# NVlabs/nvbio

Hardware: NVIDIA H100
Metric: Mreads/s (150bp) seed+extend (higher is better)
Workload: dtype int32

## Files before the change

nvbio_b200/csrc/gotoh_kernels.cu:

```cuda
#include "gotoh_core.cuh"
#include <atomic>
#include "../../include/nvbio_b200_debug.h"
#include "gotoh_full_core.cuh"
#include "pipeline_core.cuh"

namespace nvb {

static int g_traceback_fast = 1;
static int g_pair_extra_smem = 0;
static int g_pair_rows2 = 1;
static bool g_pair_fmt_ok = true;

constexpr int PAIR_BLOCKDIM    = 128;
constexpr int GENERIC_BLOCKDIM = 128;

struct GotohBatch {
    StrSet   pat, txt;
    const uint8_t* quals;
    const uint32_t* d_n;
    uint32_t n_max;
    int32_t* score;
    uint2*   sink;
};

// ... 15 lines not shown
            b.txt.words, b.txt.bits, b.txt.big_endian, str_off(b.txt, a), str_len(b.txt, a));
        b.score[a] = r.score;
        b.sink[a]  = make_uint2(r.x, r.y);
    }
}

template <int B, int TYPE>
__global__ void __launch_bounds__(GENERIC_BLOCKDIM)
gotoh_best2_kernel(const GotohScheme S, const GotohBatch b, uint32_t distinct_dist, int32_t* __restrict__ out6)
{
    const uint32_t n = batch_count(b);
    const uint32_t a = blockIdx.x * GENERIC_BLOCKDIM + threadIdx.x;
    if (a >= n) return;
    Best2 b2; b2.init(distinct_dist);
    gotoh_generic_impl<B, TYPE, false>(S, b.pat.words, b.pat.bits, b.pat.big_endian, str_off(b.pat, a), str_len(b.pat, a), b.quals,
                                       b.txt.words, b.txt.bits, b.txt.big_endian, str_off(b.txt, a), str_len(b.txt, a), nullptr, &b2);
    int32_t* o = out6 + 6 * (size_t)a;
    o[0] = b2.s1; o[1] = (int32_t)b2.x1; o[2] = (int32_t)b2.y1; o[3] = b2.s2; o[4] = (int32_t)b2.x2; o[5] = (int32_t)b2.y2;
}
template <int B, int TYPE>
static int launch_best2(const GotohScheme& S, const GotohBatch& b, uint32_t distinct_dist, int32_t* out6, cudaStream_t s)
{
    gotoh_best2_kernel<B, TYPE><<<(b.n_max + GENERIC_BLOCKDIM - 1) / GENERIC_BLOCKDIM, GENERIC_BLOCKDIM, 0, s>>>(S, b, distinct_dist, out6);
    NVB_LAUNCH_CHECK();
    return NVB_OK;
}

__device__ __forceinline__ uint32_t swap_2bit_order(uint32_t x) {
    const uint32_t r = __brev(x);
    return ((r >> 1) & 0x55555555u) | ((r & 0x55555555u) << 1);
}

template <int B, int TYPE, int PFMT, bool ROWS2>
__global__ void __launch_bounds__(PAIR_BLOCKDIM, 4)
gotoh_pair_kernel(const GotohScheme S, const GotohBatch b, uint32_t sel_rows, uint32_t* __restrict__ todo, uint32_t* __restrict__ todo_count)
{
    extern __shared__ uint16_t sel_smem[];
    __shared__ uint32_t prof_tab[256];
    for (uint32_t q = threadIdx.x; q < 256u; q += PAIR_BLOCKDIM) prof_tab[q] = sub_profile(q, S.match - S.pgo, S.mismatch - S.pgo);
    __syncthreads();
    const uint32_t n = batch_count(b);
    const uint32_t n_pairs = (n + 1u) / 2u;
    uint16_t* my_sel = sel_smem + threadIdx.x;
    {
        const uint32_t pair = blockIdx.x * PAIR_BLOCKDIM + threadIdx.x;
        if (pair >= n_pairs) return;
        const uint32_t a0 = 2u * pair;
        const bool has1 = (a0 + 1u < n);
        const uint32_t a1 = has1 ? a0 + 1u : a0;

        const uint32_t M0 = str_len(b.pat, a0), M1 = str_len(b.pat, a1);
        const uint32_t N0 = str_len(b.txt, a0), N1 = str_len(b.txt, a1);
        const uint32_t Mmax = M0 > M1 ? M0 : M1;
        const uint32_t L = Mmax + (uint32_t)B - 1u;

        const bool ok = (M0 >= 1u) && (M1 >= 1u) && (N0 >= M0 + (uint32_t)B - 1u) && (N1 >= M1 + (uint32_t)B - 1u) &&
                        (L <= sel_rows) && (TYPE == NVB_LOCAL || M0 == M1);
        if (!ok) {
            const uint32_t cnt = has1 ? 2u : 1u;
            const uint32_t slot = atomicAdd(todo_count, cnt);
            todo[slot] = a0;
            if (has1) todo[slot + 1u] = a1;
            return;
        }

        {
            const uint32_t t0 = str_off(b.txt, a0), t1 = str_off(b.txt, a1);
            const uint32_t* __restrict__ w = b.txt.words;
            const bool be = b.txt.big_endian != 0;
            const uint32_t w0 = t0 >> 4, w1 = t1 >> 4;
            const uint32_t sh0 = 2u * (t0 & 15u), sh1 = 2u * (t1 & 15u);
            const uint32_t last0 = (t0 + N0 - 1u) >> 4, last1 = (t1 + N1 - 1u) >> 4;
            const uint32_t nw = (L + 15u) >> 4;
            for (uint32_t kb = 0; kb < nw; kb += 8u) {
                uint32_t a0[9], a1[9];
#pragma unroll
                for (uint32_t q = 0; q < 9u; ++q) {
                    a0[q] = (w0 + kb + q <= last0) ? w[w0 + kb + q] : 0u;
                    a1[q] = (w1 + kb + q <= last1) ? w[w1 + kb + q] : 0u;
                }
#pragma unroll
                for (uint32_t q = 0; q < 8u; ++q) {
                    const uint32_t k = kb + q;
                    if (k < nw) {
                        uint32_t c0, c1;
                        if (be) {
                            c0 = sh0 ? ((a0[q] << sh0) | (a0[q + 1] >> (32u - sh0))) : a0[q];
                            c1 = sh1 ? ((a1[q] << sh1) | (a1[q + 1] >> (32u - sh1))) : a1[q];
                        } else {
                            c0 = sh0 ? ((a0[q] >> sh0) | (a0[q + 1] << (32u - sh0))) : a0[q];
                            c1 = sh1 ? ((a1[q] >> sh1) | (a1[q + 1] << (32u - sh1))) : a1[q];
                        }
                        const uint32_t first = k << 4;
                        const uint32_t v0 = N0 > first ? (N0 - first < 16u ? N0 - first : 16u) : 0u;
                        const uint32_t v1 = N1 > first ? (N1 - first < 16u ? N1 - first : 16u) : 0u;
                        const uint32_t m0 = v0 >= 16u ? 0xFFFFFFFFu : (be ? ~(0xFFFFFFFFu >> (2u * v0)) : ((1u << (2u * v0)) - 1u));
                        const uint32_t m1 = v1 >= 16u ? 0xFFFFFFFFu : (be ? ~(0xFFFFFFFFu >> (2u * v1)) : ((1u << (2u * v1)) - 1u));
                        c0 &= m0; c1 &= m1;
                        if (!be) { c0 = swap_2bit_order(c0); c1 = swap_2bit_order(c1); }
#pragma unroll
                        for (uint32_t by = 0; by < 4u; ++by) {
                            const uint32_t W = prmt(c0, c1, (3u - by) | ((7u - by) << 4) | 0x3200u);
#pragma unroll
                            for (uint32_t m = 0; m < 4u; ++m) {
                                const uint32_t x = (W >> (6u - 2u * m)) & 0x0303u;
                                my_sel[(first + 4u * by + m) * PAIR_BLOCKDIM] = (uint16_t)(x * 0x11u + 0xC480u);
                            }
                        }
                    }
                }
            }
        }

        SinkResult r0, r1;
        gotoh_pair<B, TYPE, PFMT, ROWS2>(S, b.pat.words, b.pat.bits, b.pat.big_endian,
                            str_off(b.pat, a0), M0, str_off(b.pat, a1), M1, N0, N1,
                            my_sel, PAIR_BLOCKDIM, r0, r1, b.quals, prof_tab);
        b.score[a0] = r0.score; b.sink[a0] = make_uint2(r0.x, r0.y);
        if (has1) { b.score[a1] = r1.score; b.sink[a1] = make_uint2(r1.x, r1.y); }
    }
}

template <int TYPE>
__global__ void __launch_bounds__(GENERIC_BLOCKDIM)
gotoh_full_kernel(const GotohScheme S, const GotohBatch b, int2* __restrict__ col)
{
    const uint32_t n = batch_count(b);
    const uint32_t a = blockIdx.x * GENERIC_BLOCKDIM + threadIdx.x;
    if (a >= n) return;
    const SinkResult r = gotoh_full<TYPE>(S, b.pat.words, b.pat.bits, b.pat.big_endian, str_off(b.pat, a), str_len(b.pat, a),
                                          b.txt.words, b.txt.bits, b.txt.big_endian, str_off(b.txt, a), str_len(b.txt, a),
                                          col + a, (size_t)b.n_max, b.quals);
    b.score[a] = r.score;
    b.sink[a]  = make_uint2(r.x, r.y);
}

struct WindowArgs { uint32_t wb, we; const int32_t* min_score; short2* ckpt; uint8_t* alive; };

template <int B, int TYPE>
__global__ void __launch_bounds__(GENERIC_BLOCKDIM)
gotoh_window_kernel(const GotohScheme S, const GotohBatch b, const WindowArgs w)
{
    const uint32_t n = batch_count(b);
    const uint32_t a = blockIdx.x * GENERIC_BLOCKDIM + threadIdx.x;
    if (a >= n) return;
    SinkResult r;
    if (w.wb == 0) { r.score = NVB_SINK_MIN; r.x = r.y = 0xFFFFFFFFu; b.score[a] = r.score; b.sink[a] = make_uint2(r.x, r.y); w.alive[a] = 1; }
    else { if (!w.alive[a]) return; r.score = b.score[a]; const uint2 k = b.sink[a]; r.x = k.x; r.y = k.y; }
    const uint32_t M = str_len(b.pat, a);
    if (w.wb >= M) return;
    const bool ok = gotoh_window<B, TYPE>(S, b.pat.words, b.pat.bits, b.pat.big_endian, str_off(b.pat, a), M, b.quals,
                                          b.txt.words, b.txt.bits, b.txt.big_endian, str_off(b.txt, a), str_len(b.txt, a),
// ... 361 lines not shown
    }
    const uint32_t lane = threadIdx.x & 31u, a0 = a - lane;
    const uint32_t wrote = __ballot_sync(0xffffffffu, done);
    for (uint32_t w = wrote; w; w &= w - 1u) {
        const uint32_t src = __ffs(w) - 1u;
        uint32_t m = __shfl_sync(0xffffffffu, len, src);
        m = m < o.max_ops ? m : o.max_ops;
        uint8_t* ops = o.ops + (size_t)(a0 + src) * o.max_ops;
        for (uint32_t i = lane; i < m; i += 32u) ops[i] = (uint8_t)DIR_SUB;
    }
}

template <int B, int TYPE>
static int launch_traceback(const GotohScheme& S, const GotohBatch& b, const TracebackOut& o, const uint32_t* todo, const uint32_t* todo_count, cudaStream_t s)
{
    const uint32_t grid = (b.n_max + GENERIC_BLOCKDIM - 1) / GENERIC_BLOCKDIM;
    gotoh_traceback_kernel<B, TYPE><<<grid, GENERIC_BLOCKDIM, 0, s>>>(S, b, o, todo, todo_count);
    NVB_LAUNCH_CHECK();
    return NVB_OK;
}

template <int B, int TYPE>
static int launch_generic(const GotohScheme& S, const GotohBatch& b, const uint32_t* todo, const uint32_t* todo_count, uint32_t n_hint, cudaStream_t s)
{
    uint32_t grid = (n_hint + GENERIC_BLOCKDIM - 1) / GENERIC_BLOCKDIM;
    const uint32_t cap = sm_count() * 32u;
    if (todo) grid = grid < cap ? grid : cap;
    if (grid == 0) grid = 1;
    gotoh_generic_kernel<B, TYPE><<<grid, GENERIC_BLOCKDIM, 0, s>>>(S, b, todo, todo_count);
    NVB_LAUNCH_CHECK();
    return NVB_OK;
}

template <int B, int TYPE, int PFMT, bool ROWS2>
static int launch_pair_fmt(const GotohScheme& S, const GotohBatch& b, uint32_t sel_rows, uint32_t* todo, uint32_t* todo_count, cudaStream_t s)
{
    const size_t smem = (size_t)((sel_rows + 15u) & ~15u) * PAIR_BLOCKDIM * sizeof(uint16_t) + (size_t)g_pair_extra_smem;
    static std::atomic<bool> attr_done[NVB_MAX_DEVICES];
    int dev = 0;
    NVB_CUDA_TRY(cudaGetDevice(&dev));
    if (dev < 0 || dev >= NVB_MAX_DEVICES) return NVB_E_UNSUPPORTED;
    if (!attr_done[dev].load(std::memory_order_acquire)) {
        NVB_CUDA_TRY(cudaFuncSetAttribute(gotoh_pair_kernel<B, TYPE, PFMT, ROWS2>, cudaFuncAttributeMaxDynamicSharedMemorySize, 200 * 1024));
        attr_done[dev].store(true, std::memory_order_release);
    }
    const uint32_t pairs = (b.n_max + 1u) / 2u;
    const uint32_t grid = (pairs + PAIR_BLOCKDIM - 1) / PAIR_BLOCKDIM;
    gotoh_pair_kernel<B, TYPE, PFMT, ROWS2><<<grid, PAIR_BLOCKDIM, smem, s>>>(S, b, sel_rows, todo, todo_count);
    NVB_LAUNCH_CHECK();
    return NVB_OK;
}
template <int B, int TYPE, int PFMT>
static int launch_pair_rows(const GotohScheme& S, const GotohBatch& b, uint32_t sel_rows, uint32_t* todo, uint32_t* todo_count, cudaStream_t s)
{
    if (g_pair_rows2) return launch_pair_fmt<B, TYPE, PFMT, true>(S, b, sel_rows, todo, todo_count, s);
    return launch_pair_fmt<B, TYPE, PFMT, false>(S, b, sel_rows, todo, todo_count, s);
}
template <int B, int TYPE>
static int launch_pair(const GotohScheme& S, const GotohBatch& b, uint32_t sel_rows, uint32_t* todo, uint32_t* todo_count, cudaStream_t s)
{
    if (!S.qtab && b.pat.big_endian && b.pat.bits == 2u && g_pair_fmt_ok) return launch_pair_rows<B, TYPE, 2>(S, b, sel_rows, todo, todo_count, s);
    if (!S.qtab && b.pat.big_endian && b.pat.bits == 4u && g_pair_fmt_ok) return launch_pair_rows<B, TYPE, 4>(S, b, sel_rows, todo, todo_count, s);
    return launch_pair_rows<B, TYPE, 0>(S, b, sel_rows, todo, todo_count, s);
}

#define NVB_TYPE_SWITCH(BAND, FN, ...)                                            \
    switch (type) {                                                               \
    case NVB_GLOBAL:      return FN<BAND, NVB_GLOBAL>(__VA_ARGS__);               \
    case NVB_LOCAL:       return FN<BAND, NVB_LOCAL>(__VA_ARGS__);                \
    case NVB_SEMI_GLOBAL: return FN<BAND, NVB_SEMI_GLOBAL>(__VA_ARGS__);          \
    default:              return NVB_E_INVALID; }

static int dispatch_generic(int band, int type, const GotohScheme& S, const GotohBatch& b, const uint32_t* todo, const uint32_t* todo_count, uint32_t n_hint, cudaStream_t s)
{
    switch (band) {
    case 3:  NVB_TYPE_SWITCH(3,  launch_generic, S, b, todo, todo_count, n_hint, s)
    case 5:  NVB_TYPE_SWITCH(5,  launch_generic, S, b, todo, todo_count, n_hint, s)
    case 7:  NVB_TYPE_SWITCH(7,  launch_generic, S, b, todo, todo_count, n_hint, s)
    case 15: NVB_TYPE_SWITCH(15, launch_generic, S, b, todo, todo_count, n_hint, s)
    case 31: NVB_TYPE_SWITCH(31, launch_generic, S, b, todo, todo_count, n_hint, s)
    case 63: NVB_TYPE_SWITCH(63, launch_generic, S, b, todo, todo_count, n_hint, s)
    }
    return NVB_E_INVALID;
// ... 30 lines not shown
static void set_route(int packed, const uint32_t* todo_count) { g_route_packed = packed; g_route_todo_count = todo_count; }

static int banded_impl(int band, int type, const nvb_gotoh_scheme* scheme,
                       const nvb_string_set* patterns, const uint8_t* d_quals, const nvb_string_set* texts,
                       const uint32_t* d_n, uint32_t n_max, int32_t* d_score, nvb_uint2* d_sink,
                       void* d_temp, size_t* temp_bytes, void* stream)
{
    if (!scheme || !temp_bytes || !valid_strset(patterns) || !valid_strset(texts)) return NVB_E_INVALID;
    if (!(band == 3 || band == 5 || band == 7 || band == 15 || band == 31 || band == 63)) return NVB_E_INVALID;
    if (type < 0 || type > 2) return NVB_E_INVALID;

    TempCarver tc(d_temp);
    uint32_t* todo_count = tc.take<uint32_t>(4);
    uint32_t* todo       = tc.take<uint32_t>((size_t)n_max + 2);
    const size_t need = tc.total();
    if (!d_temp || *temp_bytes < need) { *temp_bytes = need; return NVB_E_TEMP_SIZE; }
    if (n_max == 0) return NVB_OK;
    if (!d_score || !d_sink) return NVB_E_INVALID;

    cudaStream_t s = as_stream(stream);
    GotohBatch b;
    b.pat = make_strset(patterns); b.txt = make_strset(texts); b.quals = d_quals;
    b.d_n = d_n; b.n_max = n_max; b.score = d_score; b.sink = (uint2*)d_sink;
    const GotohScheme S = make_scheme(scheme);

    const uint32_t max_m = patterns->length;
    const uint32_t sel_rows = max_m + (uint32_t)band - 1u;
    const size_t smem = (size_t)((sel_rows + 15u) & ~15u) * PAIR_BLOCKDIM * sizeof(uint16_t);
    const bool fast = (g_force_path != 1) && texts->bits == 2 && max_m >= 1 && smem <= 200u * 1024u &&
                      pair_path_ok(band, type, scheme, max_m);
    if (!fast) { set_route(0, nullptr); return dispatch_generic(band, type, S, b, nullptr, nullptr, n_max, s); }

    set_route(1, todo_count);
    NVB_CUDA_TRY(cudaMemsetAsync(todo_count, 0, sizeof(uint32_t), s));
    int r = dispatch_pair(band, type, S, b, sel_rows, todo, todo_count, s);
    if (r != NVB_OK) return r;
    return dispatch_generic(band, type, S, b, todo, todo_count, n_max, s);
}

template <int TYPE, int W>
static int full_tb_launch(const FullTbArgs* a, uint32_t max_n, size_t* pool_bytes, cudaStream_t s)
{
    int per_sm = 0;
    NVB_CUDA_TRY(cudaOccupancyMaxActiveBlocksPerMultiprocessor(&per_sm, gotoh_full_warp_traceback_kernel<TYPE, W>, WARP_BLOCKDIM, 0));
    const uint32_t grid = sm_count() * (uint32_t)(per_sm > 0 ? per_sm : 1);
    const uint32_t slot_words = (max_n + 31u) * 32u * (uint32_t)FullTbLane<W>::NW;
    *pool_bytes = (size_t)grid * (WARP_BLOCKDIM / 32) * slot_words * sizeof(uint32_t);
    if (!a) return NVB_OK;
    gotoh_full_warp_traceback_kernel<TYPE, W><<<grid, WARP_BLOCKDIM, 0, s>>>(a->S, a->pat, a->txt, a->quals, a->score, a->sink, a->items,
                                                                            a->n_items, a->o, (uint32_t*)a->pool, slot_words);
    NVB_LAUNCH_CHECK();
    return NVB_OK;
}

int full_warp_traceback(int type, uint32_t max_m, uint32_t max_n, const FullTbArgs* a, size_t* pool_bytes, cudaStream_t s)
{
    if (max_m < 1u || max_m > FULL_TB_MAX_M || max_n > 65535u) return NVB_E_UNSUPPORTED;
#define NVB_TB_W(T)                                                                                                                 \
    switch ((max_m + 31u) / 32u) {                                                                                                  \
    case 1:  return full_tb_launch<T, 1>(a, max_n, pool_bytes, s);  case 2:  return full_tb_launch<T, 2>(a, max_n, pool_bytes, s);   \
    case 3:  return full_tb_launch<T, 3>(a, max_n, pool_bytes, s);  case 4:  return full_tb_launch<T, 4>(a, max_n, pool_bytes, s);   \
    case 5:  return full_tb_launch<T, 5>(a, max_n, pool_bytes, s);  case 6:  return full_tb_launch<T, 6>(a, max_n, pool_bytes, s);   \
    case 7:  return full_tb_launch<T, 7>(a, max_n, pool_bytes, s);  case 8:  return full_tb_launch<T, 8>(a, max_n, pool_bytes, s);   \
    case 9:  return full_tb_launch<T, 9>(a, max_n, pool_bytes, s);  case 10: return full_tb_launch<T, 10>(a, max_n, pool_bytes, s);  \
    case 11: return full_tb_launch<T, 11>(a, max_n, pool_bytes, s); case 12: return full_tb_launch<T, 12>(a, max_n, pool_bytes, s);  \
    case 13: return full_tb_launch<T, 13>(a, max_n, pool_bytes, s); case 14: return full_tb_launch<T, 14>(a, max_n, pool_bytes, s);  \
    case 15: return full_tb_launch<T, 15>(a, max_n, pool_bytes, s); default: return full_tb_launch<T, 16>(a, max_n, pool_bytes, s); }
// ... 346 lines not shown
```

nvbio_b200/csrc/pipeline.cu:

```cuda
#include "fm_core.cuh"
#include "gotoh_core.cuh"
#include "pipeline_core.cuh"
#include "gotoh_full_core.cuh"
#include <cub/agent/single_pass_scan_operators.cuh>
#include <cub/block/block_scan.cuh>
#include <cub/device/device_scan.cuh>
#include <cub/device/device_segmented_sort.cuh>
#include <mutex>

namespace nvb {

struct PipeGeom {
    uint32_t n_reads;
    uint32_t n_strings;
    uint32_t strands;
    uint32_t stride;
    uint32_t bits;
    uint32_t seeds_per_string;
    uint32_t seed_len, seed_interval;
    uint32_t band;
    uint32_t max_seed_hits;
    uint32_t genome_len;
};

// ... 172 lines not shown
    }
}

__global__ void __launch_bounds__(256)
pipe_expand_hits_kernel(const FmIndex f, const PipeGeom g, const uint2* __restrict__ ranges, const uint32_t* __restrict__ sizes,
                        const uint32_t* __restrict__ excl, const uint32_t* __restrict__ slen, const uint32_t* __restrict__ counts,
                        uint32_t* __restrict__ hit_string, uint32_t* __restrict__ p_off, uint32_t* __restrict__ p_len,
                        uint32_t* __restrict__ t_off, uint32_t* __restrict__ t_len)
{
    const uint32_t q = blockIdx.x * 256 + threadIdx.x;
    if (q >= g.n_strings * g.seeds_per_string) return;
    const uint32_t sz = sizes[q];
    if (sz == 0) return;
    const uint32_t base = excl[q], kept = counts[0];
    const uint32_t x = ranges[q].x;
    const uint32_t s = q / g.seeds_per_string, k = q % g.seeds_per_string;
    const uint32_t seed_begin = k * g.seed_interval;
    const uint32_t len = slen[s];
    for (uint32_t j = 0; j < sz; ++j) {
        const uint32_t h = base + j;
        if (h >= kept) break;
        const uint2 w = hit_window(fm_locate_one(f, x + j), seed_begin, len, g);
        hit_string[h] = s;
        p_off[h] = s * g.stride; p_len[h] = len;
        t_off[h] = w.x;          t_len[h] = w.y - w.x;
    }
}

struct Jobs { uint32_t *p_off, *p_len, *t_off, *t_len; };

constexpr uint32_t RJ_BLOCK = 128;
constexpr uint32_t RJ_STAGE = 640;
constexpr int      RJ_LOCAL = 6;
constexpr uint32_t RJ_CLAIMED = 0xFFFFFFFFu, RJ_CLAIMED_EMPTY = 0xFFFFFFFEu;
using RjTileState = cub::ScanTileState<uint32_t>;
using RjPrefixOp  = cub::TilePrefixCallbackOp<uint32_t, ::cuda::std::plus<uint32_t>, RjTileState>;

__global__ void __launch_bounds__(256)
pipe_resolve_init_kernel(RjTileState tiles, const uint32_t n_tiles, uint32_t* __restrict__ counts, uint32_t* __restrict__ dp_count)
{
    tiles.InitializeStatus((int)n_tiles);
    if (blockIdx.x == 0 && threadIdx.x == 0) { counts[2] = 0u; counts[3] = 0u; *dp_count = 0u; }
}

__global__ void __launch_bounds__(RJ_BLOCK, 8)
pipe_resolve_reads_kernel(const FmIndex f, const PipeGeom g, const uint2* __restrict__ ranges, const uint32_t* __restrict__ slen,
                          const uint32_t hit_capacity, RjTileState tiles, const uint32_t n_tiles, uint32_t* __restrict__ counts,
                          const int shortcut, const int32_t match, const int32_t mismatch, const int32_t max_gap_open,
                          const uint32_t* __restrict__ str_words, const uint32_t* __restrict__ genome,
                          uint32_t* __restrict__ j_string, uint32_t* __restrict__ j_first, const Jobs jobs,
                          int32_t* __restrict__ job_score, uint2* __restrict__ job_sink,
                          const Jobs dp, uint32_t* __restrict__ dp_job, uint32_t* __restrict__ dp_count,
                          unsigned long long* __restrict__ best_key, int32_t* best_score, uint32_t* best_pos, uint8_t* __restrict__ best_strand)
{
    using BlockScan = cub::BlockScan<uint32_t, RJ_BLOCK>;
    __shared__ struct { typename RjPrefixOp::TempStorage prefix; typename BlockScan::TempStorage scan; } s_tmp;
    __shared__ uint32_t st_string[RJ_STAGE], st_first[RJ_STAGE], st_toff[RJ_STAGE], st_tlen[RJ_STAGE], st_slot[RJ_STAGE];
    __shared__ unsigned long long s_key[RJ_BLOCK];
    __shared__ int32_t s_score[RJ_BLOCK];
    __shared__ uint32_t s_pos[RJ_BLOCK];
    __shared__ uint8_t s_strand[RJ_BLOCK];
    __shared__ uint32_t s_tile, s_cnt, s_base, s_dp_cnt, s_dp_base;
    if (threadIdx.x == 0) { s_tile = atomicAdd(counts + 3, 1u); s_cnt = 0u; s_dp_cnt = 0u; }
    s_key[threadIdx.x] = 0ull;
    __syncthreads();
    const uint32_t tile = s_tile, r0 = tile * RJ_BLOCK, r = r0 + threadIdx.x;
    const uint32_t per_read = g.strands * g.seeds_per_string;
    const bool live = r < g.n_reads;
    const uint2* rr = ranges + (size_t)r * per_read;

    uint32_t hits = 0, run = 0;
    if (live)
        for (uint32_t q = 0; q < per_read; ++q) hits += seed_range_hits(rr[q], g.max_seed_hits);
    if (tile == 0) {
        uint32_t aggregate;
        BlockScan(s_tmp.scan).ExclusiveSum(hits, run, aggregate);
        if (threadIdx.x == 0) tiles.SetInclusive(0, aggregate);
    } else {
        RjPrefixOp prefix(tiles, s_tmp.prefix, ::cuda::std::plus<uint32_t>{}, (int)tile);
        BlockScan(s_tmp.scan).ExclusiveSum(hits, run, prefix);
    }
    if (tile == n_tiles - 1u && threadIdx.x == RJ_BLOCK - 1u) {
        const uint32_t total = run + hits;
        counts[1] = total;
        counts[0] = total < hit_capacity ? total : hit_capacity;
    }

    if (live) {
        uint32_t lk_s[RJ_LOCAL], lk_b[RJ_LOCAL], lk_e[RJ_LOCAL];
        int n_local = 0;
        for (uint32_t strand = 0; strand < g.strands; ++strand) {
            const uint32_t s = r * g.strands + strand;
            const uint32_t len = slen[s];
            for (uint32_t k = 0; k < g.seeds_per_string; ++k) {
                const uint2 rq = rr[strand * g.seeds_per_string + k];
                const bool located = rq.y == 0xFFFFFFFFu;
                const uint32_t sz = seed_range_hits(rq, g.max_seed_hits);
                if (sz == 0u) continue;
                const uint32_t base = run, x = rq.x, seed_begin = k * g.seed_interval;
                run += sz;
                for (uint32_t j = 0; j < sz; ++j) {
                    const uint32_t h = base + j;
                    if (h >= hit_capacity) break;
                    const uint2 w = hit_window(located ? x : fm_locate_one(f, x + j), seed_begin, len, g);
                    bool seen = false;
#pragma unroll
                    for (int e = 0; e < RJ_LOCAL; ++e) seen |= (e < n_local) && lk_s[e] == s && lk_b[e] == w.x && lk_e[e] == w.y;
                    if (seen) continue;
#pragma unroll
                    for (int e = 0; e < RJ_LOCAL; ++e) if (e == n_local) { lk_s[e] = s; lk_b[e] = w.x; lk_e[e] = w.y; }
                    if (n_local < RJ_LOCAL) ++n_local;
                    const uint32_t slot = atomicAdd(&s_cnt, 1u);
                    if (slot < RJ_STAGE) { st_string[slot] = s; st_first[slot] = h; st_toff[slot] = w.x; st_tlen[slot] = w.y - w.x; }
                    else {
                        const uint32_t o = atomicAdd(counts + 2, 1u), d = atomicAdd(dp_count, 1u);
                        j_string[o] = s; j_first[o] = h;
                        jobs.p_off[o] = s * g.stride; jobs.p_len[o] = len; jobs.t_off[o] = w.x; jobs.t_len[o] = w.y - w.x;
                        dp.p_off[d] = s * g.stride; dp.p_len[d] = len; dp.t_off[d] = w.x; dp.t_len[d] = w.y - w.x; dp_job[d] = o;
                    }
                }
            }
        }
    }
    __syncthreads();

    const uint32_t n = s_cnt < RJ_STAGE ? s_cnt : RJ_STAGE;
    if (threadIdx.x == 0) s_base = n ? atomicAdd(counts + 2, n) : 0u;
    __syncthreads();
    for (uint32_t i = threadIdx.x; i < n; i += RJ_BLOCK) {
        const uint32_t o = s_base + i, s = st_string[i], first = st_first[i], len = slen[s], to = st_toff[i], N = st_tlen[i];
        j_string[o] = s; j_first[o] = first; jobs.p_off[o] = s * g.stride; jobs.p_len[o] = len; jobs.t_off[o] = to; jobs.t_len[o] = N;
        int32_t score = 0; uint32_t sx = 0, sy = 0;
        if (shortcut && gapless_job_shortcut(str_words, genome, s * g.stride, len, to, N, g.band, match, mismatch, max_gap_open, score, sx, sy,
                                             shortcut != 2)) {
            const uint2 sk = make_uint2(sx, sy);
            job_score[o] = score; job_sink[o] = sk;
            if (job_aligned(sk)) {
                st_slot[i] = RJ_CLAIMED; st_toff[i] = to + sx; st_tlen[i] = (uint32_t)score;
                atomicMax(&s_key[s / g.strands - r0], make_best_key(score, first));
            } else st_slot[i] = RJ_CLAIMED_EMPTY;
        } else st_slot[i] = atomicAdd(&s_dp_cnt, 1u);
    }
    __syncthreads();
    if (threadIdx.x == 0) s_dp_base = s_dp_cnt ? atomicAdd(dp_count, s_dp_cnt) : 0u;
    __syncthreads();
    for (uint32_t i = threadIdx.x; i < n; i += RJ_BLOCK) {
        const uint32_t slot = st_slot[i], s = st_string[i];
        if (slot == RJ_CLAIMED) {
            const uint32_t rl = s / g.strands - r0;
            const int32_t score = (int32_t)st_tlen[i];
            if (s_key[rl] == make_best_key(score, st_first[i])) { s_score[rl] = score; s_pos[rl] = st_toff[i]; s_strand[rl] = (uint8_t)(s % g.strands); }
// ... 1203 lines not shown
```

nvbio_b200/csrc/pipeline_core.cuh:

```cuda
#pragma once
#include "fm_core.cuh"

namespace nvb {

__host__ __device__ __forceinline__ uint32_t nvb_clz(uint32_t x) {
#ifdef __CUDA_ARCH__
    return (uint32_t)__clz((int)x);
#else
    return (uint32_t)__builtin_clz(x);
#endif
}

__host__ __device__ __forceinline__ uint32_t job_diff_bits(const uint32_t* __restrict__ str_words, const uint32_t* __restrict__ genome,
                                                           const uint32_t po, const uint32_t t, const uint32_t i, const uint32_t cnt)
{
    const uint32_t x = (be2_window(str_words, po + i, cnt) ^ be2_window(genome, t + i, cnt)) >> (32u - 2u * cnt);
    return (x | (x >> 1)) & 0x55555555u;
}
__host__ __device__ __forceinline__ uint32_t job_differences(const uint32_t* __restrict__ str_words, const uint32_t* __restrict__ genome,
                                                             const uint32_t po, const uint32_t M, const uint32_t t, const uint32_t limit)
{
    uint32_t mm = 0;
    for (uint32_t i = 0; i < M && mm <= limit; i += 16u) mm += nvb_popc(job_diff_bits(str_words, genome, po, t, i, M - i < 16u ? M - i : 16u));
    return mm;
}

__host__ __device__ __forceinline__ uint32_t diff_row_mask(const uint32_t w0, const uint32_t cnt, const uint32_t lo, const uint32_t hi)
{
    const uint32_t a = lo > w0 ? lo : w0, b = hi < w0 + cnt - 1u ? hi : w0 + cnt - 1u;
    if (a > b) return 0u;
    return ((2u << (2u * (w0 + cnt - 1u - a))) - 1u) & ~((1u << (2u * (w0 + cnt - 1u - b))) - 1u);
}
__host__ __device__ inline void job_diff_span(const uint32_t* __restrict__ str_words, const uint32_t* __restrict__ genome, const uint32_t po,
                                              const uint32_t t, const uint32_t lo, const uint32_t hi, int32_t& first, int32_t& last)
{
    first = (int32_t)hi + 1; last = (int32_t)lo - 1;
    for (uint32_t i = lo; i <= hi; i += 16u) {
        const uint32_t cnt = hi + 1u - i < 16u ? hi + 1u - i : 16u;
        const uint32_t d = job_diff_bits(str_words, genome, po, t, i, cnt);
        if (!d) continue;
        if (first > (int32_t)hi) first = (int32_t)(i + cnt - 1u - ((31u - nvb_clz(d)) >> 1));
        last = (int32_t)(i + cnt - 1u - ((31u - nvb_clz(d & (0u - d))) >> 1));
    }
}
__host__ __device__ __forceinline__ uint32_t text_window16(const uint32_t g0, const uint32_t g1, const uint32_t g2, const uint32_t g3, const uint32_t off)
{
    const uint32_t idx = off >> 4, sh = 2u * (off & 15u);
    const uint32_t hi = idx == 0u ? g0 : (idx == 1u ? g1 : g2), lo = idx == 0u ? g1 : (idx == 1u ? g2 : g3);
    return sh ? ((hi << sh) | (lo >> (32u - sh))) : hi;
}

__host__ __device__ inline bool gapless_job_shortcut(const uint32_t* __restrict__ str_words, const uint32_t* __restrict__ genome,
                                                     const uint32_t po, const uint32_t M, const uint32_t to, const uint32_t N, const uint32_t band,
                                                     const int32_t match, const int32_t mismatch, const int32_t max_gap_open,
                                                     int32_t& score, uint32_t& sink_x, uint32_t& sink_y, const bool one_gap = true)
{
    if (M < 1u || to == 0u || N < M + band - 1u) return false;
    const uint32_t j0 = band / 2u;
    const int32_t o = -max_gap_open, lim = !one_gap ? o : (o + match - mismatch < 2 * o ? o + match - mismatch : 2 * o);
    const uint32_t mm_max = (uint32_t)((lim - 1) / match);
    int32_t h = 0, best = 0, f1 = (int32_t)M, f2 = (int32_t)M, l1 = -1, l2 = -1; uint32_t end = 0, prev = 0, mm0 = 0;
    for (uint32_t i = 0; i < M && mm0 <= mm_max; i += 16u) {
        const uint32_t cnt = M - i < 16u ? M - i : 16u;
        uint32_t d = job_diff_bits(str_words, genome, po, to + j0, i, cnt);
        while (d && mm0 <= mm_max) {
            const uint32_t bit = 31u - nvb_clz(d);
            const uint32_t p = i + (cnt - 1u - (bit >> 1));
            d &= ~(1u << bit);
            h += match * (int32_t)(p - prev);
            if (h >= best) { best = h; end = p; }
            h += mismatch; h = h > 0 ? h : 0;
            if (mm0 == 0u) f1 = (int32_t)p; else if (mm0 == 1u) f2 = (int32_t)p;
            l2 = l1; l1 = (int32_t)p;
            prev = p + 1u; ++mm0;
        }
    }
    if (mm0 > mm_max) return false;
    h += match * (int32_t)(M - prev);
    if (h >= best) { best = h; end = M; }
    const int32_t delta = match * (int32_t)M - best;
    if (delta >= lim) return false;
    const bool gap1 = delta >= o;
    const uint32_t U = gap1 ? (uint32_t)((delta - o) / match) : 0u;
    if (gap1 && 2u * U + 1u > M) return false;
    const uint32_t hi = M - 1u - U;
    int32_t fa = f1 >= (int32_t)U ? f1 : (f2 >= (int32_t)U ? f2 : (int32_t)(M - U)), ba = l1 <= (int32_t)hi ? l1 : (l2 <= (int32_t)hi ? l2 : (int32_t)U - 1);
    fa = fa > (int32_t)hi ? (int32_t)(M - U) : fa; ba = ba < (int32_t)U ? (int32_t)U - 1 : ba;
    int32_t fb = INT_MIN, bb = INT_MAX; uint32_t fd = j0, bd = j0;
    const bool perfect = (mm0 == 0u);
    const uint32_t t = (uint32_t)(delta / match);
    const uint32_t c16 = M < 16u ? M : 16u;
    const uint32_t r0 = be2_window(str_words, po, c16) >> (32u - 2u * c16);
    const uint32_t wi = to >> 4, r = to & 15u, wl = (to + N - 1u) >> 4;
    const uint32_t g0 = genome[wi], g1 = (wi + 1u <= wl) ? genome[wi + 1u] : 0u;
    const uint32_t g2 = (wi + 2u <= wl) ? genome[wi + 2u] : 0u, g3 = (wi + 3u <= wl) ? genome[wi + 3u] : 0u;
    uint32_t rE = 0, e0 = 0, e1 = 0, e2 = 0, e3 = 0, mF = 0, mB = 0;
    const uint32_t te = to + M - c16, we = te >> 4;
    if (gap1) {
        rE = be2_window(str_words, po + M - c16, c16) >> (32u - 2u * c16);
        e0 = genome[we]; e1 = (we + 1u <= wl) ? genome[we + 1u] : 0u; e2 = (we + 2u <= wl) ? genome[we + 2u] : 0u; e3 = (we + 3u <= wl) ? genome[we + 3u] : 0u;
        mF = diff_row_mask(0u, c16, U, hi); mB = diff_row_mask(M - c16, c16, U, hi);
    }
    uint32_t jtop = j0;
    for (uint32_t jj = 0; jj < band; ++jj) {
        if (jj == j0) continue;
        const uint32_t x = (text_window16(g0, g1, g2, g3, r + jj) >> (32u - 2u * c16)) ^ r0, dx = (x | (x >> 1)) & 0x55555555u;
        if (gap1) {
// ... 176 lines not shown
```

Before: 400.2.

## Add persistent ticket scheduling to pair kernel, batch seed range loads, prefetch shortcut words

The pair Gotoh kernel gains a persistent-grid mode, used when the batch count lives on the device: warps claim 32 pairs at a time from an atomic ticket counter and the grid is capped at resident occupancy. The resolve-jobs kernel now loads seed ranges in vectorized batches and walks only non-empty ranges via bitmasks. The gapless shortcut prefetches read and genome words into registers and computes diffs inline instead of calling a per-16-base helper. Together these aim to cut wasted blocks, scalar loads and latency, at the cost of more register pressure and a second counter word that must be zeroed.

```diff
diff --git a/nvbio_b200/csrc/gotoh_kernels.cu b/nvbio_b200/csrc/gotoh_kernels.cu
--- a/nvbio_b200/csrc/gotoh_kernels.cu
+++ b/nvbio_b200/csrc/gotoh_kernels.cu
@@ -71,6 +71,86 @@
 }
 
 template <int B, int TYPE, int PFMT, bool ROWS2>
+__device__ __forceinline__ void gotoh_pair_job(const GotohScheme& S, const GotohBatch& b, const uint32_t sel_rows, uint32_t* __restrict__ todo,
+                                               uint32_t* __restrict__ todo_count, const uint32_t pair, const uint32_t n, uint16_t* my_sel,
+                                               const uint32_t* prof_tab)
+{
+    const uint32_t a0 = 2u * pair;
+    const bool has1 = (a0 + 1u < n);
+    const uint32_t a1 = has1 ? a0 + 1u : a0;
+
+    const uint32_t M0 = str_len(b.pat, a0), M1 = str_len(b.pat, a1);
+    const uint32_t N0 = str_len(b.txt, a0), N1 = str_len(b.txt, a1);
+    const uint32_t Mmax = M0 > M1 ? M0 : M1;
+    const uint32_t L = Mmax + (uint32_t)B - 1u;
+
+    const bool ok = (M0 >= 1u) && (M1 >= 1u) && (N0 >= M0 + (uint32_t)B - 1u) && (N1 >= M1 + (uint32_t)B - 1u) &&
+                    (L <= sel_rows) && (TYPE == NVB_LOCAL || M0 == M1);
+    if (!ok) {
+        const uint32_t cnt = has1 ? 2u : 1u;
+        const uint32_t slot = atomicAdd(todo_count, cnt);
+        todo[slot] = a0;
+        if (has1) todo[slot + 1u] = a1;
+        return;
+    }
+
+    {
+        const uint32_t t0 = str_off(b.txt, a0), t1 = str_off(b.txt, a1);
+        const uint32_t* __restrict__ w = b.txt.words;
+        const bool be = b.txt.big_endian != 0;
+        const uint32_t w0 = t0 >> 4, w1 = t1 >> 4;
+        const uint32_t sh0 = 2u * (t0 & 15u), sh1 = 2u * (t1 & 15u);
+        const uint32_t last0 = (t0 + N0 - 1u) >> 4, last1 = (t1 + N1 - 1u) >> 4;
+        const uint32_t nw = (L + 15u) >> 4;
+        for (uint32_t kb = 0; kb < nw; kb += 8u) {
+            uint32_t a0[9], a1[9];
+#pragma unroll
+            for (uint32_t q = 0; q < 9u; ++q) {
+                a0[q] = (w0 + kb + q <= last0) ? w[w0 + kb + q] : 0u;
+                a1[q] = (w1 + kb + q <= last1) ? w[w1 + kb + q] : 0u;
+            }
+#pragma unroll
+            for (uint32_t q = 0; q < 8u; ++q) {
+                const uint32_t k = kb + q;
+                if (k < nw) {
+                    uint32_t c0, c1;
+                    if (be) {
+                        c0 = sh0 ? ((a0[q] << sh0) | (a0[q + 1] >> (32u - sh0))) : a0[q];
+                        c1 = sh1 ? ((a1[q] << sh1) | (a1[q + 1] >> (32u - sh1))) : a1[q];
+                    } else {
+                        c0 = sh0 ? ((a0[q] >> sh0) | (a0[q + 1] << (32u - sh0))) : a0[q];
+                        c1 = sh1 ? ((a1[q] >> sh1) | (a1[q + 1] << (32u - sh1))) : a1[q];
+                    }
+                    const uint32_t first = k << 4;
+                    const uint32_t v0 = N0 > first ? (N0 - first < 16u ? N0 - first : 16u) : 0u;
+                    const uint32_t v1 = N1 > first ? (N1 - first < 16u ? N1 - first : 16u) : 0u;
+                    const uint32_t m0 = v0 >= 16u ? 0xFFFFFFFFu : (be ? ~(0xFFFFFFFFu >> (2u * v0)) : ((1u << (2u * v0)) - 1u));
+                    const uint32_t m1 = v1 >= 16u ? 0xFFFFFFFFu : (be ? ~(0xFFFFFFFFu >> (2u * v1)) : ((1u << (2u * v1)) - 1u));
+                    c0 &= m0; c1 &= m1;
+                    if (!be) { c0 = swap_2bit_order(c0); c1 = swap_2bit_order(c1); }
+#pragma unroll
+                    for (uint32_t by = 0; by < 4u; ++by) {
+                        const uint32_t W = prmt(c0, c1, (3u - by) | ((7u - by) << 4) | 0x3200u);
+#pragma unroll
+                        for (uint32_t m = 0; m < 4u; ++m) {
+                            const uint32_t x = (W >> (6u - 2u * m)) & 0x0303u;
+                            my_sel[(first + 4u * by + m) * PAIR_BLOCKDIM] = (uint16_t)(x * 0x11u + 0xC480u);
+                        }
+                    }
+                }
+            }
+        }
+    }
+
+    SinkResult r0, r1;
+    gotoh_pair<B, TYPE, PFMT, ROWS2>(S, b.pat.words, b.pat.bits, b.pat.big_endian,
+                        str_off(b.pat, a0), M0, str_off(b.pat, a1), M1, N0, N1,
+                        my_sel, PAIR_BLOCKDIM, r0, r1, b.quals, prof_tab);
+    b.score[a0] = r0.score; b.sink[a0] = make_uint2(r0.x, r0.y);
+    if (has1) { b.score[a1] = r1.score; b.sink[a1] = make_uint2(r1.x, r1.y); }
+}
+
+template <int B, int TYPE, int PFMT, bool ROWS2, bool TICKET>
 __global__ void __launch_bounds__(PAIR_BLOCKDIM, 4)
 gotoh_pair_kernel(const GotohScheme S, const GotohBatch b, uint32_t sel_rows, uint32_t* __restrict__ todo, uint32_t* __restrict__ todo_count)
 {
@@ -81,82 +161,19 @@
     const uint32_t n = batch_count(b);
     const uint32_t n_pairs = (n + 1u) / 2u;
     uint16_t* my_sel = sel_smem + threadIdx.x;
-    {
+    if (!TICKET) {
         const uint32_t pair = blockIdx.x * PAIR_BLOCKDIM + threadIdx.x;
         if (pair >= n_pairs) return;
-        const uint32_t a0 = 2u * pair;
-        const bool has1 = (a0 + 1u < n);
-        const uint32_t a1 = has1 ? a0 + 1u : a0;
-
-        const uint32_t M0 = str_len(b.pat, a0), M1 = str_len(b.pat, a1);
-        const uint32_t N0 = str_len(b.txt, a0), N1 = str_len(b.txt, a1);
-        const uint32_t Mmax = M0 > M1 ? M0 : M1;
-        const uint32_t L = Mmax + (uint32_t)B - 1u;
-
-        const bool ok = (M0 >= 1u) && (M1 >= 1u) && (N0 >= M0 + (uint32_t)B - 1u) && (N1 >= M1 + (uint32_t)B - 1u) &&
-                        (L <= sel_rows) && (TYPE == NVB_LOCAL || M0 == M1);
-        if (!ok) {
-            const uint32_t cnt = has1 ? 2u : 1u;
-            const uint32_t slot = atomicAdd(todo_count, cnt);
-            todo[slot] = a0;
-            if (has1) todo[slot + 1u] = a1;
-            return;
-        }
-
-        {
-            const uint32_t t0 = str_off(b.txt, a0), t1 = str_off(b.txt, a1);
-            const uint32_t* __restrict__ w = b.txt.words;
-            const bool be = b.txt.big_endian != 0;
-            const uint32_t w0 = t0 >> 4, w1 = t1 >> 4;
-            const uint32_t sh0 = 2u * (t0 & 15u), sh1 = 2u * (t1 & 15u);
-            const uint32_t last0 = (t0 + N0 - 1u) >> 4, last1 = (t1 + N1 - 1u) >> 4;
-            const uint32_t nw = (L + 15u) >> 4;
-            for (uint32_t kb = 0; kb < nw; kb += 8u) {
-                uint32_t a0[9], a1[9];
-#pragma unroll
-                for (uint32_t q = 0; q < 9u; ++q) {
-                    a0[q] = (w0 + kb + q <= last0) ? w[w0 + kb + q] : 0u;
-                    a1[q] = (w1 + kb + q <= last1) ? w[w1 + kb + q] : 0u;
-                }
-#pragma unroll
-                for (uint32_t q = 0; q < 8u; ++q) {
-                    const uint32_t k = kb + q;
-                    if (k < nw) {
-                        uint32_t c0, c1;
-                        if (be) {
-                            c0 = sh0 ? ((a0[q] << sh0) | (a0[q + 1] >> (32u - sh0))) : a0[q];
-                            c1 = sh1 ? ((a1[q] << sh1) | (a1[q + 1] >> (32u - sh1))) : a1[q];
-                        } else {
-                            c0 = sh0 ? ((a0[q] >> sh0) | (a0[q + 1] << (32u - sh0))) : a0[q];
-                            c1 = sh1 ? ((a1[q] >> sh1) | (a1[q + 1] << (32u - sh1))) : a1[q];
-                        }
-                        const uint32_t first = k << 4;
-                        const uint32_t v0 = N0 > first ? (N0 - first < 16u ? N0 - first : 16u) : 0u;
-                        const uint32_t v1 = N1 > first ? (N1 - first < 16u ? N1 - first : 16u) : 0u;
-                        const uint32_t m0 = v0 >= 16u ? 0xFFFFFFFFu : (be ? ~(0xFFFFFFFFu >> (2u * v0)) : ((1u << (2u * v0)) - 1u));
-                        const uint32_t m1 = v1 >= 16u ? 0xFFFFFFFFu : (be ? ~(0xFFFFFFFFu >> (2u * v1)) : ((1u << (2u * v1)) - 1u));
-                        c0 &= m0; c1 &= m1;
-                        if (!be) { c0 = swap_2bit_order(c0); c1 = swap_2bit_order(c1); }
-#pragma unroll
-                        for (uint32_t by = 0; by < 4u; ++by) {
-                            const uint32_t W = prmt(c0, c1, (3u - by) | ((7u - by) << 4) | 0x3200u);
-#pragma unroll
-                            for (uint32_t m = 0; m < 4u; ++m) {
-                                const uint32_t x = (W >> (6u - 2u * m)) & 0x0303u;
-                                my_sel[(first + 4u * by + m) * PAIR_BLOCKDIM] = (uint16_t)(x * 0x11u + 0xC480u);
-                            }
-                        }
-                    }
-                }
-            }
-        }
-
-        SinkResult r0, r1;
-        gotoh_pair<B, TYPE, PFMT, ROWS2>(S, b.pat.words, b.pat.bits, b.pat.big_endian,
-                            str_off(b.pat, a0), M0, str_off(b.pat, a1), M1, N0, N1,
-                            my_sel, PAIR_BLOCKDIM, r0, r1, b.quals, prof_tab);
-        b.score[a0] = r0.score; b.sink[a0] = make_uint2(r0.x, r0.y);
-        if (has1) { b.score[a1] = r1.score; b.sink[a1] = make_uint2(r1.x, r1.y); }
+        gotoh_pair_job<B, TYPE, PFMT, ROWS2>(S, b, sel_rows, todo, todo_count, pair, n, my_sel, prof_tab);
+    } else {
+        const uint32_t lane = threadIdx.x & 31u;
+        for (;;) {
+            uint32_t first = 0;
+            if (lane == 0u) first = atomicAdd(todo_count + 1, 32u);
+            first = __shfl_sync(0xFFFFFFFFu, first, 0);
+            if (first >= n_pairs) return;
+            if (first + lane < n_pairs) gotoh_pair_job<B, TYPE, PFMT, ROWS2>(S, b, sel_rows, todo, todo_count, first + lane, n, my_sel, prof_tab);
+        }
     }
 }
 
@@ -584,8 +601,8 @@
     return NVB_OK;
 }
 
-template <int B, int TYPE, int PFMT, bool ROWS2>
-static int launch_pair_fmt(const GotohScheme& S, const GotohBatch& b, uint32_t sel_rows, uint32_t* todo, uint32_t* todo_count, cudaStream_t s)
+template <int B, int TYPE, int PFMT, bool ROWS2, bool TICKET>
+static int launch_pair_grid(const GotohScheme& S, const GotohBatch& b, uint32_t sel_rows, uint32_t* todo, uint32_t* todo_count, cudaStream_t s)
 {
     const size_t smem = (size_t)((sel_rows + 15u) & ~15u) * PAIR_BLOCKDIM * sizeof(uint16_t) + (size_t)g_pair_extra_smem;
     static std::atomic<bool> attr_done[NVB_MAX_DEVICES];
@@ -593,14 +610,26 @@
     NVB_CUDA_TRY(cudaGetDevice(&dev));
     if (dev < 0 || dev >= NVB_MAX_DEVICES) return NVB_E_UNSUPPORTED;
     if (!attr_done[dev].load(std::memory_order_acquire)) {
-        NVB_CUDA_TRY(cudaFuncSetAttribute(gotoh_pair_kernel<B, TYPE, PFMT, ROWS2>, cudaFuncAttributeMaxDynamicSharedMemorySize, 200 * 1024));
+        NVB_CUDA_TRY(cudaFuncSetAttribute(gotoh_pair_kernel<B, TYPE, PFMT, ROWS2, TICKET>, cudaFuncAttributeMaxDynamicSharedMemorySize, 200 * 1024));
         attr_done[dev].store(true, std::memory_order_release);
     }
     const uint32_t pairs = (b.n_max + 1u) / 2u;
-    const uint32_t grid = (pairs + PAIR_BLOCKDIM - 1) / PAIR_BLOCKDIM;
-    gotoh_pair_kernel<B, TYPE, PFMT, ROWS2><<<grid, PAIR_BLOCKDIM, smem, s>>>(S, b, sel_rows, todo, todo_count);
+    uint32_t grid = (pairs + PAIR_BLOCKDIM - 1) / PAIR_BLOCKDIM;
+    if (TICKET) {
+        int per_sm = 0;
+        NVB_CUDA_TRY(cudaOccupancyMaxActiveBlocksPerMultiprocessor(&per_sm, gotoh_pair_kernel<B, TYPE, PFMT, ROWS2, TICKET>, PAIR_BLOCKDIM, smem));
+        const uint32_t resident = sm_count() * (uint32_t)(per_sm > 0 ? per_sm : 1);
+        grid = grid < resident ? grid : resident;
+    }
+    gotoh_pair_kernel<B, TYPE, PFMT, ROWS2, TICKET><<<grid, PAIR_BLOCKDIM, smem, s>>>(S, b, sel_rows, todo, todo_count);
     NVB_LAUNCH_CHECK();
     return NVB_OK;
+}
+template <int B, int TYPE, int PFMT, bool ROWS2>
+static int launch_pair_fmt(const GotohScheme& S, const GotohBatch& b, uint32_t sel_rows, uint32_t* todo, uint32_t* todo_count, cudaStream_t s)
+{
+    if (b.d_n) return launch_pair_grid<B, TYPE, PFMT, ROWS2, true>(S, b, sel_rows, todo, todo_count, s);
+    return launch_pair_grid<B, TYPE, PFMT, ROWS2, false>(S, b, sel_rows, todo, todo_count, s);
 }
 template <int B, int TYPE, int PFMT>
 static int launch_pair_rows(const GotohScheme& S, const GotohBatch& b, uint32_t sel_rows, uint32_t* todo, uint32_t* todo_count, cudaStream_t s)
@@ -697,7 +726,7 @@
     if (!fast) { set_route(0, nullptr); return dispatch_generic(band, type, S, b, nullptr, nullptr, n_max, s); }
 
     set_route(1, todo_count);
-    NVB_CUDA_TRY(cudaMemsetAsync(todo_count, 0, sizeof(uint32_t), s));
+    NVB_CUDA_TRY(cudaMemsetAsync(todo_count, 0, 2 * sizeof(uint32_t), s));
     int r = dispatch_pair(band, type, S, b, sel_rows, todo, todo_count, s);
     if (r != NVB_OK) return r;
     return dispatch_generic(band, type, S, b, todo, todo_count, n_max, s);
diff --git a/nvbio_b200/csrc/pipeline.cu b/nvbio_b200/csrc/pipeline.cu
--- a/nvbio_b200/csrc/pipeline.cu
+++ b/nvbio_b200/csrc/pipeline.cu
@@ -228,9 +228,35 @@
 constexpr uint32_t RJ_BLOCK = 128;
 constexpr uint32_t RJ_STAGE = 640;
 constexpr int      RJ_LOCAL = 6;
+constexpr uint32_t RJ_BATCH = 4;
 constexpr uint32_t RJ_CLAIMED = 0xFFFFFFFFu, RJ_CLAIMED_EMPTY = 0xFFFFFFFEu;
 using RjTileState = cub::ScanTileState<uint32_t>;
 using RjPrefixOp  = cub::TilePrefixCallbackOp<uint32_t, ::cuda::std::plus<uint32_t>, RjTileState>;
+
+template <uint32_t RB>
+__device__ __forceinline__ uint32_t range_batch(const uint2* __restrict__ rr, const uint32_t q0, const uint32_t n, const bool vec,
+                                                const uint32_t max_seed_hits, uint32_t& hits)
+{
+    uint2 v[RB];
+    if (vec) {
+#pragma unroll
+        for (uint32_t j = 0; j < RB; j += 2u) {
+            const uint4 w = q0 + j < n ? *reinterpret_cast<const uint4*>(rr + q0 + j) : make_uint4(1u, 0u, 1u, 0u);
+            v[j] = make_uint2(w.x, w.y); v[j + 1] = make_uint2(w.z, w.w);
+        }
+    } else {
+#pragma unroll
+        for (uint32_t j = 0; j < RB; ++j) v[j] = q0 + j < n ? rr[q0 + j] : make_uint2(1u, 0u);
+    }
+    uint32_t m = 0;
+#pragma unroll
+    for (uint32_t j = 0; j < RB; ++j) {
+        const uint32_t sz = seed_range_hits(v[j], max_seed_hits);
+        hits += sz;
+        m |= (sz != 0u ? 1u : 0u) << j;
+    }
+    return m;
+}
 
 __global__ void __launch_bounds__(256)
 pipe_resolve_init_kernel(RjTileState tiles, const uint32_t n_tiles, uint32_t* __restrict__ counts, uint32_t* __restrict__ dp_count)
@@ -265,9 +291,13 @@
     const bool live = r < g.n_reads;
     const uint2* rr = ranges + (size_t)r * per_read;
 
-    uint32_t hits = 0, run = 0;
+    const bool vec = ((per_read | (uint32_t)((size_t)ranges >> 3)) & 1u) == 0u;
+    uint32_t hits = 0, run = 0, nonempty = 0;
     if (live)
-        for (uint32_t q = 0; q < per_read; ++q) hits += seed_range_hits(rr[q], g.max_seed_hits);
+        for (uint32_t q0 = 0; q0 < per_read; q0 += 16u) {
+            const uint32_t m = range_batch<16>(rr, q0, per_read, vec, g.max_seed_hits, hits);
+            if (q0 < 32u) nonempty |= m << q0;
+        }
     if (tile == 0) {
         uint32_t aggregate;
         BlockScan(s_tmp.scan).ExclusiveSum(hits, run, aggregate);
@@ -285,34 +315,48 @@
     if (live) {
         uint32_t lk_s[RJ_LOCAL], lk_b[RJ_LOCAL], lk_e[RJ_LOCAL];
         int n_local = 0;
-        for (uint32_t strand = 0; strand < g.strands; ++strand) {
-            const uint32_t s = r * g.strands + strand;
-            const uint32_t len = slen[s];
-            for (uint32_t k = 0; k < g.seeds_per_string; ++k) {
-                const uint2 rq = rr[strand * g.seeds_per_string + k];
-                const bool located = rq.y == 0xFFFFFFFFu;
-                const uint32_t sz = seed_range_hits(rq, g.max_seed_hits);
-                if (sz == 0u) continue;
-                const uint32_t base = run, x = rq.x, seed_begin = k * g.seed_interval;
-                run += sz;
-                for (uint32_t j = 0; j < sz; ++j) {
-                    const uint32_t h = base + j;
-                    if (h >= hit_capacity) break;
-                    const uint2 w = hit_window(located ? x : fm_locate_one(f, x + j), seed_begin, len, g);
-                    bool seen = false;
+        const uint32_t len0 = slen[r * g.strands], len1 = g.strands > 1u ? slen[r * g.strands + 1u] : 0u;
+        for (uint32_t q0 = 0; q0 < per_read; q0 += 32u) {
+            uint32_t m = q0 ? 0u : nonempty, unused = 0;
+            if (q0)
+                for (uint32_t b = 0; b < 32u; b += 8u) m |= range_batch<8>(rr, q0 + b, per_read, vec, g.max_seed_hits, unused) << b;
+            while (m) {
+                uint32_t bq[RJ_BATCH], nb = 0;
+                uint2 brq[RJ_BATCH];
 #pragma unroll
-                    for (int e = 0; e < RJ_LOCAL; ++e) seen |= (e < n_local) && lk_s[e] == s && lk_b[e] == w.x && lk_e[e] == w.y;
-                    if (seen) continue;
+                for (uint32_t e = 0; e < RJ_BATCH; ++e) { bq[e] = m ? q0 + (uint32_t)__ffs(m) - 1u : 0u; nb += m ? 1u : 0u; m &= m - 1u; }
 #pragma unroll
-                    for (int e = 0; e < RJ_LOCAL; ++e) if (e == n_local) { lk_s[e] = s; lk_b[e] = w.x; lk_e[e] = w.y; }
-                    if (n_local < RJ_LOCAL) ++n_local;
-                    const uint32_t slot = atomicAdd(&s_cnt, 1u);
-                    if (slot < RJ_STAGE) { st_string[slot] = s; st_first[slot] = h; st_toff[slot] = w.x; st_tlen[slot] = w.y - w.x; }
-                    else {
-                        const uint32_t o = atomicAdd(counts + 2, 1u), d = atomicAdd(dp_count, 1u);
-                        j_string[o] = s; j_first[o] = h;
-                        jobs.p_off[o] = s * g.stride; jobs.p_len[o] = len; jobs.t_off[o] = w.x; jobs.t_len[o] = w.y - w.x;
-                        dp.p_off[d] = s * g.stride; dp.p_len[d] = len; dp.t_off[d] = w.x; dp.t_len[d] = w.y - w.x; dp_job[d] = o;
+                for (uint32_t e = 0; e < RJ_BATCH; ++e) brq[e] = e < nb ? rr[bq[e]] : make_uint2(1u, 0u);
+                for (uint32_t e = 0; e < nb; ++e) {
+                    const uint32_t q = bq[0];
+                    const uint2 rq = brq[0];
+#pragma unroll
+                    for (uint32_t c = 0; c + 1u < RJ_BATCH; ++c) { bq[c] = bq[c + 1]; brq[c] = brq[c + 1]; }
+                    const uint32_t strand = q < g.seeds_per_string ? 0u : 1u, k = q - strand * g.seeds_per_string;
+                    const uint32_t s = r * g.strands + strand, len = strand ? len1 : len0;
+                    const bool located = rq.y == 0xFFFFFFFFu;
+                    const uint32_t sz = seed_range_hits(rq, g.max_seed_hits);
+                    const uint32_t base = run, x = rq.x, seed_begin = k * g.seed_interval;
+                    run += sz;
+                    for (uint32_t j = 0; j < sz; ++j) {
+                        const uint32_t h = base + j;
+                        if (h >= hit_capacity) break;
+                        const uint2 w = hit_window(located ? x : fm_locate_one(f, x + j), seed_begin, len, g);
+                        bool seen = false;
+#pragma unroll
+                        for (int e = 0; e < RJ_LOCAL; ++e) seen |= (e < n_local) && lk_s[e] == s && lk_b[e] == w.x && lk_e[e] == w.y;
+                        if (seen) continue;
+#pragma unroll
+                        for (int e = 0; e < RJ_LOCAL; ++e) if (e == n_local) { lk_s[e] = s; lk_b[e] = w.x; lk_e[e] = w.y; }
+                        if (n_local < RJ_LOCAL) ++n_local;
+                        const uint32_t slot = atomicAdd(&s_cnt, 1u);
+                        if (slot < RJ_STAGE) { st_string[slot] = s; st_first[slot] = h; st_toff[slot] = w.x; st_tlen[slot] = w.y - w.x; }
+                        else {
+                            const uint32_t o = atomicAdd(counts + 2, 1u), d = atomicAdd(dp_count, 1u);
+                            j_string[o] = s; j_first[o] = h;
+                            jobs.p_off[o] = s * g.stride; jobs.p_len[o] = len; jobs.t_off[o] = w.x; jobs.t_len[o] = w.y - w.x;
+                            dp.p_off[d] = s * g.stride; dp.p_len[d] = len; dp.t_off[d] = w.x; dp.t_len[d] = w.y - w.x; dp_job[d] = o;
+                        }
                     }
                 }
             }
diff --git a/nvbio_b200/csrc/pipeline_core.cuh b/nvbio_b200/csrc/pipeline_core.cuh
--- a/nvbio_b200/csrc/pipeline_core.cuh
+++ b/nvbio_b200/csrc/pipeline_core.cuh
@@ -50,6 +50,8 @@
     return sh ? ((hi << sh) | (lo >> (32u - sh))) : hi;
 }
 
+constexpr uint32_t SHORTCUT_WORDS = 10;
+
 __host__ __device__ inline bool gapless_job_shortcut(const uint32_t* __restrict__ str_words, const uint32_t* __restrict__ genome,
                                                      const uint32_t po, const uint32_t M, const uint32_t to, const uint32_t N, const uint32_t band,
                                                      const int32_t match, const int32_t mismatch, const int32_t max_gap_open,
@@ -60,19 +62,31 @@
     const int32_t o = -max_gap_open, lim = !one_gap ? o : (o + match - mismatch < 2 * o ? o + match - mismatch : 2 * o);
     const uint32_t mm_max = (uint32_t)((lim - 1) / match);
     int32_t h = 0, best = 0, f1 = (int32_t)M, f2 = (int32_t)M, l1 = -1, l2 = -1; uint32_t end = 0, prev = 0, mm0 = 0;
-    for (uint32_t i = 0; i < M && mm0 <= mm_max; i += 16u) {
-        const uint32_t cnt = M - i < 16u ? M - i : 16u;
-        uint32_t d = job_diff_bits(str_words, genome, po, to + j0, i, cnt);
-        while (d && mm0 <= mm_max) {
-            const uint32_t bit = 31u - nvb_clz(d);
-            const uint32_t p = i + (cnt - 1u - (bit >> 1));
-            d &= ~(1u << bit);
-            h += match * (int32_t)(p - prev);
-            if (h >= best) { best = h; end = p; }
-            h += mismatch; h = h > 0 ? h : 0;
-            if (mm0 == 0u) f1 = (int32_t)p; else if (mm0 == 1u) f2 = (int32_t)p;
-            l2 = l1; l1 = (int32_t)p;
-            prev = p + 1u; ++mm0;
+    const uint32_t wr = po >> 4, wt = (to + j0) >> 4, sht = 2u * ((to + j0) & 15u), wlast = (to + N - 1u) >> 4;
+    for (uint32_t kb = 0; kb * 16u < M && mm0 <= mm_max; kb += SHORTCUT_WORDS) {
+        uint32_t rw[SHORTCUT_WORDS], tw[SHORTCUT_WORDS + 1];
+#pragma unroll
+        for (uint32_t q = 0; q < SHORTCUT_WORDS; ++q) rw[q] = (kb + q) * 16u < M ? str_words[wr + kb + q] : 0u;
+#pragma unroll
+        for (uint32_t q = 0; q <= SHORTCUT_WORDS; ++q) tw[q] = wt + kb + q <= wlast ? genome[wt + kb + q] : 0u;
+#pragma unroll
+        for (uint32_t q = 0; q < SHORTCUT_WORDS; ++q) {
+            const uint32_t i = (kb + q) * 16u;
+            if (i >= M || mm0 > mm_max) break;
+            const uint32_t cnt = M - i < 16u ? M - i : 16u;
+            const uint32_t x = (rw[q] ^ (sht ? (tw[q] << sht) | (tw[q + 1] >> (32u - sht)) : tw[q])) >> (32u - 2u * cnt);
+            uint32_t d = (x | (x >> 1)) & 0x55555555u;
+            while (d && mm0 <= mm_max) {
+                const uint32_t bit = 31u - nvb_clz(d);
+                const uint32_t p = i + (cnt - 1u - (bit >> 1));
+                d &= ~(1u << bit);
+                h += match * (int32_t)(p - prev);
+                if (h >= best) { best = h; end = p; }
+                h += mismatch; h = h > 0 ? h : 0;
+                if (mm0 == 0u) f1 = (int32_t)p; else if (mm0 == 1u) f2 = (int32_t)p;
+                l2 = l1; l1 = (int32_t)p;
+                prev = p + 1u; ++mm0;
+            }
         }
     }
     if (mm0 > mm_max) return false;
```

Result: faster. 430.1, median of 6 (+7.5%).
